# robertknight/rten

Measured on NVIDIA H100. Metric: resnet50_fp32_inferences_per_sec, higher is better.
Workload: dtype f32(tf32 mma, explicit opt-in)

## Files before the change

### rten_b200/csrc/umma_gemm.cu

```cuda
#include <cuda.h>
#include <cuda_runtime.h>

#include <algorithm>
#include <array>
#include <cmath>
#include <vector>
#include <cmath>
#include <cstdint>
#include <cstdio>
#include <cstdlib>

#include "math.cuh"
#include "ptx.cuh"
#include "rowops.h"
#include "umma_gemm.h"
#include "umma_kernel.cuh"

namespace rtb {

typedef CUresult (*EncodeTiledFn)(CUtensorMap*, CUtensorMapDataType, cuuint32_t, void*, const cuuint64_t*,
                                  const cuuint64_t*, const cuuint32_t*, const cuuint32_t*, CUtensorMapInterleave,
                                  CUtensorMapSwizzle, CUtensorMapL2promotion, CUtensorMapFloatOOBfill);

static EncodeTiledFn get_encode(rten_ctx* ctx) {
// ... 38 lines not shown
        long long s = od.strides[i] * esize;
        if (s == 0 || od.dims[i] == 1) s = 16;
        strides[i - 1] = (cuuint64_t)s;
    }
    CUresult r = enc(map, is_f32 ? CU_TENSOR_MAP_DATA_TYPE_FLOAT32 : CU_TENSOR_MAP_DATA_TYPE_UINT8, 4,
                     const_cast<void*>(od.base), dims, strides, b, es, CU_TENSOR_MAP_INTERLEAVE_NONE,
                     CU_TENSOR_MAP_SWIZZLE_128B, CU_TENSOR_MAP_L2_PROMOTION_L2_256B,
                     CU_TENSOR_MAP_FLOAT_OOB_FILL_NONE);
    return r == CUDA_SUCCESS;
}

static void pick_conv_tile(const ConvGeom& g, int& tw, int& th, int& tb) {
    double best = -1.0;
    tw = th = tb = 1;
    for (int w = 1; w <= std::min(g.OW, 128); w++) {
        if (w * g.sx > 256) break;
        for (int h = 1; h <= std::min(g.OH, 128 / w); h++) {
            if (h * g.sy > 256) break;
            int b = std::min(g.B, 128 / (w * h));
            if (b < 1) continue;
            long long tiles = (long long)((g.OW + w - 1) / w) * ((g.OH + h - 1) / h) * ((g.B + b - 1) / b);
            double eff = (double)g.B * g.OH * g.OW / ((double)tiles * 128.0);
            if (eff > best + 1e-9 || (eff > best - 1e-9 && w > tw)) {
                best = eff;
                tw = w;
                th = h;
                tb = b;
            }
        }
    }
}

struct Plan {
    int bn = 32, splitk = 1, nbuf = 1;
};

struct Prepared {
    KParams p;
    uint32_t abox[4], aes[4], bbox_k;
    uint32_t pbox[4], pes[4];
    uint32_t a_rows;
    long long batch;
    OperandDesc od, ord;
    uint32_t dbox[4];
    int tma_store, res_tma;
    int wide;
    int chain_bytes;
    int step;
    int esize, kelems;
};

constexpr int SK_CNT_INTS = 1 << 16;
static int smem_budget_for(int n_stg) { return 227 * 1024 - SMEM_FIXED_BYTES - n_stg * STG_BYTES; }
static int wide_stages(int stage_bytes, int chain_bytes) {
    return std::min(MAX_STAGES, (227 * 1024 - WIDE_SMEM_FIXED_BYTES - chain_bytes) / stage_bytes);
}
static bool is_wide(int bn) { return bn > ACC_STRIDE; }

static Epi pick_epilogue(const GemmLaunch& L, int tma_store, int res_tma, int splitk) {
    const EpilogueDesc& e = L.epi;
    auto aligned = [](const void* ptr) { return (reinterpret_cast<uintptr_t>(ptr) & 15) == 0; };
    bool fast = tma_store && (L.N % 32) == 0 && !getenv("RTEN_B200_NO_FAST") && e.bias_kind != 2 &&
                (e.r == nullptr || res_tma) && (e.bias_kind != 1 || aligned(e.bias));
    if (L.kind == 1)
        fast = fast && (!(e.za || e.za8) || aligned(e.colsum)) && (!e.zb || e.zb_len == 1 || (e.zb_len == L.N && aligned(e.zb))) &&
               (!e.scale || e.scale_len == 1 || (e.scale_len == L.N && aligned(e.scale)));
    if (!fast) return Epi::Generic;
    const bool gelu = e.act > 1;
    if (!getenv("RTEN_B200_NO_PLAIN") && e.act <= 7) {
        if (L.kind == 0 && e.alpha == 1.0f && !e.range && (e.r == nullptr || e.r_scale == 1.0f))
            return gelu ? Epi::PlainF32Gelu : Epi::PlainF32;
        if (L.kind == 1 && e.scale && !e.za && !e.zb && (e.scale_len == 1 || e.scale_len == L.N) && splitk == 1 &&
            (!e.za8 || e.colsum))
            return gelu ? Epi::PlainI8Gelu : Epi::PlainI8;
    }
    return gelu ? Epi::FastGelu : Epi::Fast;
}

static const char* epi_name(Epi v) {
    static const char* const names[] = {"Generic", "Fast", "FastGelu", "PlainF32", "PlainF32Gelu", "PlainI8", "PlainI8Gelu"};
    return names[(int)v];
}

static bool is_plain_f32(Epi v) { return v == Epi::PlainF32 || v == Epi::PlainF32Gelu; }

struct PlanShape {
    long long tiles_n, units_m, tiles, units;
    int kb_per, stage_bytes, stages, n_stg;
};

static bool plan_shape(const Prepared& q, const Plan& pl, PlanShape& ps) {
    const KParams& p = q.p;
    if (pl.splitk < 1) return false;
    if (is_wide(pl.bn)) {
        if ((pl.bn != 128 && pl.bn != 256) || !q.wide || pl.splitk != 1) return false;
        if (pl.bn == 256 && q.p.epi.act > 1) return false;
    } else if (pl.bn < 16 || pl.bn % 32 || pl.bn % q.step) {
        return false;
    }
    if (pl.nbuf < (q.res_tma ? 2 : 1) || pl.nbuf > 4) return false;
    ps.tiles_n = q.chain_bytes ? 1 : (p.N + pl.bn - 1) / pl.bn;
    ps.units_m = p.tiles_m;
    ps.tiles = ps.units_m * ps.tiles_n * q.batch;
    ps.units = ps.tiles * pl.splitk;
    if (ps.units > 0x7FFFFFFFll) return false;
    ps.kb_per = (p.k_blocks + pl.splitk - 1) / pl.splitk;
    if (pl.splitk > 1) {
        if (pl.bn % 32 || (long long)(pl.splitk - 1) * ps.kb_per >= p.k_blocks) return false;
        if (ps.tiles * 2 > SK_CNT_INTS) return false;
    }
    ps.n_stg = 2 * pl.nbuf;
    ps.stage_bytes = A_STAGE_BYTES + pl.bn * KBYTES;
    ps.stages = is_wide(pl.bn) ? wide_stages(ps.stage_bytes, q.chain_bytes) : std::min(MAX_STAGES, smem_budget_for(ps.n_stg) / ps.stage_bytes);
    if (ps.stages < 2) return false;
    return true;
}

static double plan_cost(const Prepared& q, const Plan& pl, const PlanShape& ps, int num_sms) {
    const double active = (double)std::min<long long>(ps.units, num_sms);
    const double waves = std::ceil((double)ps.units / num_sms);
    const double bw = std::min(64.0, 7400.0 / active);
    const double mmas = 4.0;
    const double t_kb = std::max(mmas * std::max(42.0, (double)pl.bn), ps.stage_bytes / bw);
    double t_stage = std::max(t_kb, 320.0 + mmas * 42.0);
    t_stage = std::max(t_stage, 2300.0 / ps.stages);
    const double mainloop = ps.kb_per * t_stage;
    const double epi = is_wide(pl.bn) ? (pl.bn / 32.0) * 400.0 + 600.0 : (pl.bn / 32.0) * 350.0 / 2.0 + 600.0;
    double unit = (is_wide(pl.bn) ? mainloop + epi : std::max(mainloop, epi)) + 1500.0;
    double cost = waves * unit + 2500.0;
    if (pl.splitk > 1) cost += epi * (1.0 + 0.25 * pl.splitk) + 1500.0;

    return cost;
}

static void enumerate_plans(const Prepared& q, int num_sms, std::vector<std::pair<double, Plan>>& out) {
    const KParams& p = q.p;
    const int nmax = (p.N + q.step - 1) / q.step * q.step;
    static const int splits[] = {1, 2, 3, 4, 5, 6, 8, 10, 12, 16};
    for (int bn : {32, 64, 128, 256}) {
        if (bn > nmax && bn != 32) break;
        for (int sk : splits) {
            Plan pl;
            pl.bn = bn;
            pl.splitk = sk;
            if (sk > 1 && p.k_blocks / sk < 4) continue;
            const int kb_per = (p.k_blocks + sk - 1) / sk;
            pl.nbuf = (q.res_tma || kb_per < 24) ? 2 : 1;
            PlanShape ps;
            if (is_wide(bn)) {
                pl.nbuf = 2;
            } else if (pl.nbuf == 2 && !getenv("RTEN_B200_NO_NBUF3")) {
                PlanShape ps2;
                const bool ok2 = plan_shape(q, pl, ps2);
                pl.nbuf = 3;
                if (!plan_shape(q, pl, ps) || (ps.stages < 3 && !(ok2 && ps.stages == ps2.stages))) pl.nbuf = 2;
            }
            if (!plan_shape(q, pl, ps)) continue;
            if (sk > 1 && ps.tiles >= 2 * num_sms) continue;
            if (ps.stages < 2) continue;
            out.emplace_back(plan_cost(q, pl, ps, num_sms), pl);
        }
    }
    std::sort(out.begin(), out.end(), [](const std::pair<double, Plan>& x, const std::pair<double, Plan>& y) {
        return x.first < y.first;
    });
}

static rten_status prepare_launch(rten_ctx* ctx, const GemmLaunch& L, Prepared& q) {
    const int esize = L.kind == 0 ? 4 : 1;
    const int kelems = KBYTES / esize;
    if (!tma_compatible(L.a, esize, 4) || !tma_compatible(L.b, esize, 4)) return RTEN_ERR_UNSUPPORTED_VALUE;
    if (L.M <= 0 || L.N <= 0 || L.K <= 0) return RTEN_ERR_UNSUPPORTED_VALUE;
    q.esize = esize;
    q.kelems = kelems;
    KParams& p = q.p;
    memset(&p, 0, sizeof(p));
    p.M = L.M;
    p.N = L.N;
    p.K = L.K;
    p.z0 = L.z0;
    p.z1 = L.z1;
    p.kelems = kelems;
    p.conv = L.conv;
    p.epi = L.epi;
    p.c_blocks = 1;
    p.kw = 1;
    for (int i = 0; i < 4; i++) q.aes[i] = 1;
    if (L.conv) {
        const ConvGeom& g = L.g;
        pick_conv_tile(g, p.tw, p.th, p.tb);
        p.tiles_x = (g.OW + p.tw - 1) / p.tw;
        p.tiles_y = (g.OH + p.th - 1) / p.th;
        int tiles_b = (g.B + p.tb - 1) / p.tb;
        p.tiles_m = p.tiles_x * p.tiles_y * tiles_b;
        p.OH = g.OH;
        p.OW = g.OW;
        p.Bn = g.B;
        p.sy = g.sy;
        p.sx = g.sx;
        p.dy = g.dy;
        p.dx = g.dx;
        p.pt = g.pt;
        p.pl = g.pl;
// ... 147 lines not shown
    p.stages = ps.stages;
    p.sgn = L.kind == 0 ? 0 : (L.a_signed ? 1 : 0) | (L.b_signed ? 2 : 0);
    if (p.splitk > 1) {
        RTB_TRY(ensure_splitk_counters(ctx));
        if (!ws) RTB_TRY(temp_alloc(ctx, splitk_ws_bytes(ps, pl), &ws));
        p.sk_ws = reinterpret_cast<uint32_t*>(ws);
        p.sk_cnt = reinterpret_cast<int*>(ctx->sk_counters);
    }

    uint32_t bbox[4] = {(uint32_t)q.kelems, (uint32_t)p.bn, 1, 1}, bes[4] = {1, 1, 1, 1}, des[4] = {1, 1, 1, 1};
    TmaMaps m;
    if (!encode_map(ctx, &m.a, L.a, q.esize, L.kind == 0, q.abox, q.aes)) return RTEN_ERR_UNSUPPORTED_VALUE;
    if (!encode_map(ctx, &m.b, L.b, q.esize, L.kind == 0, bbox, bes)) return RTEN_ERR_UNSUPPORTED_VALUE;
    m.d = m.r = m.a2 = m.a_proj = m.b_proj = m.a2_proj = m.w2 = m.z = m.a;
    p.x3_cb = L.x3_cb;
    if (L.x3_cb && !encode_map(ctx, &m.a2, L.a_lo, q.esize, true, q.abox, q.aes)) return RTEN_ERR_UNSUPPORTED_VALUE;
    if (p.kb_proj) {
        p.x3_cb_proj = L.proj.x3_cb;
        if (!encode_map(ctx, &m.a_proj, L.proj.a, 4, true, q.pbox, q.pes) ||
            !encode_map(ctx, &m.b_proj, L.proj.b, 4, true, bbox, bes) ||
            (L.proj.x3_cb && !encode_map(ctx, &m.a2_proj, L.proj.a_lo, 4, true, q.pbox, q.pes)))
            return RTEN_ERR_UNSUPPORTED_VALUE;
    }
    if (p.tma_store && !encode_map(ctx, &m.d, q.od, 4, true, q.dbox, des)) {
        p.tma_store = 0;
        p.res_tma = 0;
        m.d = m.a;
    }
    if (p.res_tma && !encode_map(ctx, &m.r, q.ord, 4, true, q.dbox, des)) {
        p.res_tma = 0;
        m.r = m.a;
    }
    const Epi epi = pick_epilogue(L, p.tma_store, p.res_tma, p.splitk);
    if (epi == Epi::Generic && (L.kind == 1 || L.epi.act > 1)) p.res_tma = 0;
    if (q.chain_bytes) {
        const GemmLaunch::Chain& c = L.chain;
        const uint32_t wbox[4] = {32, (uint32_t)c.N2, 1, 1}, zbox[4] = {32, q.dbox[1], q.dbox[2], q.dbox[3]};
        if (epi != Epi::PlainF32 || (L.epi.r && !p.res_tma) || !encode_map(ctx, &m.w2, c.w, 4, true, wbox, des) ||
            !encode_map(ctx, &m.z, c.z, 4, true, zbox, des))
            return RTEN_ERR_UNSUPPORTED_VALUE;
        p.chain_n2 = c.N2;
        p.chain_passes = (L.N + p.bn - 1) / p.bn;
        p.chain_act = c.act;
        p.chain_bias = c.bias;
    }

    if (verbose)
        fprintf(stderr, "[umma_gemm] kind=%d conv=%d M=%d N=%d K=%d kb=%d kb_proj=%d tiles_m=%d bn=%d splitk=%d units=%d stages=%d tma_store=%d res_tma=%d nbuf=%d box=%dx%dx%d epi=%s%s\n",
                L.kind, L.conv, L.M, L.N, L.K, p.k_blocks, p.kb_proj, p.tiles_m, p.bn, p.splitk, p.units_total, p.stages,
                p.tma_store, p.res_tma, p.nbuf, p.tw, p.th, p.tb, epi_name(epi),
                p.chain_n2 == 64 ? " chain=64" : p.chain_n2 == 128 ? " chain=128" : "");
    if ((is_wide(p.bn) || p.kb_proj || L.epi.bias2) && !is_plain_f32(epi)) return RTEN_ERR_UNSUPPORTED_VALUE;
    const size_t smem_bytes = (size_t)p.stages * p.stage_bytes + q.chain_bytes +
                              (is_wide(p.bn) ? WIDE_SMEM_FIXED_BYTES : ps.n_stg * STG_BYTES + SMEM_FIXED_BYTES);
    using Kernel = void (*)(TmaMaps, KParams);
    static const Kernel narrow[2][7] = {
        {umma_gemm_kernel<0, Epi::Generic>, umma_gemm_kernel<0, Epi::Fast>, umma_gemm_kernel<0, Epi::FastGelu>,
         umma_gemm_kernel<0, Epi::PlainF32>, umma_gemm_kernel<0, Epi::PlainF32Gelu>, nullptr, nullptr},
        {umma_gemm_kernel<1, Epi::Generic>, umma_gemm_kernel<1, Epi::Fast>, umma_gemm_kernel<1, Epi::FastGelu>, nullptr,
         nullptr, umma_gemm_kernel<1, Epi::PlainI8>, umma_gemm_kernel<1, Epi::PlainI8Gelu>}};
    const Kernel kern = !is_wide(p.bn)              ? narrow[L.kind][(int)epi]
                        : p.chain_n2 == 64         ? umma_wide_kernel<Epi::PlainF32, 64>
                        : p.chain_n2 == 128        ? umma_wide_kernel<Epi::PlainF32, 128>
                        : epi == Epi::PlainF32Gelu ? umma_wide_kernel<Epi::PlainF32Gelu>
                                                   : umma_wide_kernel<Epi::PlainF32>;

    const int threads = is_wide(p.bn) ? WIDE_THREADS : NUM_THREADS;
    return launch(ctx, "umma_gemm launch", kern, {std::min(p.units_total, ctx->num_sms), threads, smem_bytes, 227 * 1024, true}, m, p);
}

static std::vector<long long> tune_key(const GemmLaunch& L, const Prepared& q) {
    const EpilogueDesc& e = L.epi;
    std::vector<long long> k = {L.kind, L.conv, L.M, L.N, L.K, L.z0, L.z1, q.tma_store, q.res_tma, e.act, e.bias_kind,
                                e.r != nullptr, (e.za != nullptr || e.za8 != nullptr), e.zb != nullptr, e.scale != nullptr,
                                L.a.strides[1], L.b.strides[1], L.x3_cb};
    if (L.conv) {
        const ConvGeom& g = L.g;
        for (long long v : {g.B, g.H, g.W, g.C, g.OH, g.OW, g.kh, g.kw, g.sy, g.sx, g.dy, g.dx, g.pt, g.pl}) k.push_back(v);
    }
    if (L.proj.C > 0) {
        const GemmLaunch::Projection& pr = L.proj;
        for (int64_t v : {(int64_t)-1, (int64_t)pr.C, (int64_t)pr.stride, (int64_t)pr.x3_cb, pr.a.dims[1], pr.a.dims[2],
                          pr.a.strides[1], pr.a.strides[2], pr.a.strides[3], pr.b.strides[1]})
            k.push_back(v);
    }
    return k;
}

static Plan plan_from_array(const std::array<int, 3>& a) {
    Plan pl;
    pl.bn = a[0];
    pl.splitk = a[1];
    pl.nbuf = a[2];
    return pl;
}

static rten_status launch_tf32x3(rten_ctx* ctx, const GemmLaunch& L0) {
    GemmLaunch L = L0;
    long long d0 = 0, d0p = 0;
    auto split = [&](const OperandDesc& src, OperandDesc& dst, int role, void* into) -> rten_status {
        const long long planes = role == 2 ? 1 : 3;
        long long dims[4], strides[4], n = planes * d0p;
        for (int i = 0; i < 4; i++) {
            dims[i] = (i > 0 && src.strides[i] == 0) ? 1 : src.dims[i];
            strides[i] = src.strides[i];
        }
        for (int i = 1; i < 4; i++) n *= dims[i];
        void* buf = into;
        if (!buf) RTB_TRY(temp_alloc(ctx, (size_t)n * 4, &buf));
        RTB_TRY(launch_tf32x3_split(ctx, (const float*)src.base, (float*)buf, dims, strides, d0p, role));
        dst = src;
        dst.base = buf;
        dst.dims[0] = planes * d0p;
        long long st = planes * d0p;
        for (int i = 1; i < 4; i++) {
            dst.strides[i] = (src.strides[i] == 0 && src.dims[i] > 1) ? 0 : st;
// ... 23 lines not shown
        }
        if (slot && *slot && !getenv("RTEN_B200_X3_NO_CACHE")) {
            b = b0;
            b.base = *slot;
            b.dims[0] = 3 * d0p;
            long long st = 3 * d0p;
            for (int i = 1; i < 4; i++) {
                const long long di = b0.strides[i] == 0 ? 1 : b0.dims[i];
                b.strides[i] = (b0.strides[i] == 0 && b0.dims[i] > 1) ? 0 : st;
                st *= di;
            }
        } else {
            RTB_TRY(split(b0, b, 1, nullptr));
        }
        const bool two_plane = d0 % 32 == 0 && tma_compatible(a0, 4, 4) && !getenv("RTEN_B200_X3_THREE_PLANES");
        if (two_plane && a_lo_base) {
            a_lo = a0;
            a_lo.base = a_lo_base;
            x3_cb = (int)(d0 / 32);
        } else if (two_plane) {
            RTB_TRY(split(a0, a_lo, 2, nullptr));
            x3_cb = (int)(d0 / 32);
        } else {
            RTB_TRY(split(a0, a, 0, nullptr));
        }
        return RTEN_OK;
    };
    RTB_TRY(split_source(L0.a, L0.b, L0.b_x3_slot, L0.a_lo_base, L.a, L.b, L.a_lo, L.x3_cb));
    if (L.conv)
        L.g.C = (int)(3 * d0p);
    L.K = L.conv ? (int)(L0.K / d0 * 3 * d0p) : (int)(3 * d0p);
    L.b_x3_slot = nullptr;
    L.a_lo_base = nullptr;
    if (L0.proj.C > 0) {
        RTB_TRY(split_source(L0.proj.a, L0.proj.b, L0.proj.b_x3_slot, nullptr, L.proj.a, L.proj.b, L.proj.a_lo, L.proj.x3_cb));
        L.proj.C = (int)(3 * d0p);
        L.proj.b_x3_slot = nullptr;
    }
    const int saved = ctx->f32_mode;
    ctx->f32_mode = RTEN_F32_TF32;
    const rten_status st = launch_umma_gemm(ctx, L);
    ctx->f32_mode = saved;
    return st;
}

rten_status launch_umma_gemm(rten_ctx* ctx, const GemmLaunch& L) {
    if (L.chain.N2 > 0) {
        if (L.kind != 0 || ctx->f32_mode != RTEN_F32_TF32 || L.x3_cb || getenv("RTEN_B200_NO_CHAIN"))
            return RTEN_ERR_UNSUPPORTED_VALUE;
        Prepared q;
        RTB_TRY(prepare_launch(ctx, L, q));
        Plan pl;
        pl.bn = 128;
        pl.nbuf = 2;
        return launch_plan(ctx, L, q, pl, getenv("RTEN_B200_VERBOSE") != nullptr);
    }
    if (L.kind == 0 && ctx->f32_mode == RTEN_F32_TF32X3) return launch_tf32x3(ctx, L);
    if (L.conv && L.kind == 0 && L.g.kh * L.g.kw > 1 && !L.x3_cb && !L.proj.C) {
        const rten_status hs = launch_umma_halo_conv(ctx, L);
        if (hs != RTEN_ERR_UNSUPPORTED_VALUE) return hs;
    }
    Prepared q;
    RTB_TRY(prepare_launch(ctx, L, q));
    const bool verbose = getenv("RTEN_B200_VERBOSE") != nullptr;
    const bool forced = getenv("RTEN_B200_FORCE_BN") || getenv("RTEN_B200_FORCE_SPLITK");
    if (!forced && !ctx->tune_cache.empty()) {
        auto hit = ctx->tune_cache.find(tune_key(L, q));
        if (hit != ctx->tune_cache.end()) {
            PlanShape ps;
            if (hit->second[0] < 0) {
                const rten_status hs = launch_umma_halo_conv(ctx, L, hit->second[1], hit->second[2]);
                if (hs != RTEN_ERR_UNSUPPORTED_VALUE) return hs;
            } else
            if (plan_shape(q, plan_from_array(hit->second), ps)) return launch_plan(ctx, L, q, plan_from_array(hit->second), verbose);
            if (verbose) fprintf(stderr, "[umma_gemm] recorded plan no longer valid for this problem: re-planning\n");
            ctx->tune_cache.erase(hit);
        }
    }
    std::vector<std::pair<double, Plan>> cands;
    enumerate_plans(q, ctx->num_sms, cands);
    if (cands.empty()) return RTEN_ERR_UNSUPPORTED_VALUE;
    Plan plan = cands[0].second;

    if (forced) {
        const char* fb = getenv("RTEN_B200_FORCE_BN");
        const char* fs = getenv("RTEN_B200_FORCE_SPLITK");
        bool found = false;
        for (const auto& c : cands) {
            const Plan& x = c.second;
            if (fb && x.bn != atoi(fb)) continue;
            if (fs && x.splitk != atoi(fs)) continue;
            plan = x;
            found = true;
            break;
        }
        if (!found) {
            ctx->forced_misses++;
            if (verbose) fprintf(stderr, "[umma_gemm] no valid plan matches the forced fields: using the model's choice\n");
            if (getenv("RTEN_B200_FORCE_STRICT"))
                return fail(ctx, RTEN_ERR_INVALID_VALUE, "no launch plan matches the forced RTEN_B200_FORCE_* fields");
        } else {
            ctx->forced_hits++;
        }
    } else if (ctx->autotune || !ctx->tune_cache.empty()) {
        const std::vector<long long> key = tune_key(L, q);
        auto it = ctx->tune_cache.find(key);
        PlanShape ps_hit;
// ... 107 lines not shown
```

### rten_b200/csrc/umma_kernel.cuh

```cuda
#pragma once
#include <cuda.h>
#include <cuda_runtime.h>

#include <cstdint>

#include "math.cuh"
#include "ptx.cuh"
#include "umma_gemm.h"

namespace rtb {

constexpr int BM = 128;
constexpr int KBYTES = 128;
constexpr int A_STAGE_BYTES = BM * KBYTES;
constexpr int ACC_STRIDE = 64;
constexpr int PRODUCER_WARP = 12;
constexpr int NUM_THREADS = 416;
constexpr int STG_BYTES = 128 * 128;
constexpr int MAX_STAGES = 8;

struct FastDiv {
    uint32_t d = 1, mul = 0, shr = 0;
    __host__ void set(int div) {
        d = (uint32_t)(div < 1 ? 1 : div);
// ... 46 lines not shown
    EpilogueDesc epi;
};

struct TileCoord {
    int n0;
    int m0;
    int z0, z1;
    int ox0, oy0, b0;
};

__device__ __forceinline__ TileCoord decode_tile(const KParams& p, int t) {
    TileCoord c;
    int n_blk, rest, m_blk, z;
    p.d_tiles_n.divmod(t, rest, n_blk);
    p.d_tiles_m.divmod(rest, z, m_blk);
    c.n0 = n_blk * p.bn;
    c.m0 = m_blk * BM;
    p.d_z0.divmod(z, c.z1, c.z0);
    c.ox0 = c.oy0 = c.b0 = 0;
    if (p.conv) {
        int xt, r2, yt, bt;
        p.d_tiles_x.divmod(m_blk, r2, xt);
        p.d_tiles_y.divmod(r2, bt, yt);
        c.ox0 = xt * p.tw;
        c.oy0 = yt * p.th;
        c.b0 = bt * p.tb;
    }
    return c;
}

__device__ __forceinline__ int4 out_coord(const KParams& p, const TileCoord& tc, int col) {
    return p.conv ? make_int4(tc.n0 + col, tc.ox0, tc.oy0, tc.b0) : make_int4(tc.n0 + col, tc.m0, tc.z0, tc.z1);
}

__device__ __forceinline__ void plain_f32_pair(uint32_t& v0, uint32_t& v1, bool res, float2 rr, float2 bb, bool relu) {
    if (res) add_f32x2(v0, v1, rr.x, rr.y);
    add_f32x2(v0, v1, bb.x, bb.y);
    if (relu) {
        v0 = __float_as_uint(fmaxf(__uint_as_float(v0), 0.0f));
        v1 = __float_as_uint(fmaxf(__uint_as_float(v1), 0.0f));
    }
}

__device__ __forceinline__ float column_bias(const EpilogueDesc& e, int n) {
    const float b = __ldg(e.bias + n);
    return e.bias2 ? __fadd_rn(b, __ldg(e.bias2 + n)) : b;
}

__device__ __forceinline__ void bulk_wait_read(int n) {
    switch (n) {
        case 0: asm volatile("cp.async.bulk.wait_group.read 0;" ::: "memory"); break;
        case 1: asm volatile("cp.async.bulk.wait_group.read 1;" ::: "memory"); break;
        case 2: asm volatile("cp.async.bulk.wait_group.read 2;" ::: "memory"); break;
        default: asm volatile("cp.async.bulk.wait_group.read 3;" ::: "memory"); break;
    }
}

__device__ __forceinline__ int f32_to_ordered(float f) {
    const int i = __float_as_int(f);
    return i >= 0 ? i : i ^ 0x7fffffff;
}
__device__ __forceinline__ void range_commit(int* range, float lo, float hi) {
#pragma unroll
    for (int o = 16; o > 0; o >>= 1) {
        lo = fminf(lo, __shfl_xor_sync(0xffffffffu, lo, o));
        hi = fmaxf(hi, __shfl_xor_sync(0xffffffffu, hi, o));
    }
    if ((threadIdx.x & 31) == 0 && lo <= hi) {
        atomicMin(&range[0], f32_to_ordered(lo));
        atomicMax(&range[1], f32_to_ordered(hi));
    }
}

__device__ __noinline__ float4 act4(float4 x, int act, float alpha, float beta) {
    if (act == 2) {
        gelu_ref_x2(x.x, x.y);
        gelu_ref_x2(x.z, x.w);
        return x;
    }
    x.x = apply_act(x.x, act, alpha, beta);
    x.y = apply_act(x.y, act, alpha, beta);
    x.z = apply_act(x.z, act, alpha, beta);
    x.w = apply_act(x.w, act, alpha, beta);
    return x;
}

__device__ __forceinline__ bool splitk_publish(const KParams& p, int t, int ks, int grp, int q, int lane, uint32_t t_acc,
                                               int* flag, uint32_t acc_smem) {
    const int r = q * 32 + lane;
    const int nchunks = p.bn >> 5;
    for (int c0 = grp * 32; c0 < p.bn; c0 += 64) {
        uint32_t v[32];
        acc_ld(acc_smem, t_acc + c0, v);
        uint32_t* w = p.sk_ws + ((((size_t)t * p.splitk + ks) * nchunks + (c0 >> 5)) << 12) + r;
#pragma unroll
        for (int j = 0; j < 32; j++) __stcg(w + j * 128, v[j]);
    }
    __threadfence();
    asm volatile("bar.sync %0, 128;" ::"r"(1 + grp) : "memory");
    if (q == 0 && lane == 0) {
        int* cnt = p.sk_cnt + t * 2 + grp;
        const int old = atomicAdd(cnt, 1);
        const int last = old == p.splitk - 1;
        if (last) *cnt = 0;
        __threadfence();
        *flag = last;
    }
// ... 215 lines not shown
    L.smem = base + 4096 + ACC_SMEM_BYTES;
    return L;
}

__device__ __forceinline__ void kernel_setup(const SmemLayout& L) {
    const int warp = threadIdx.x >> 5;
    const int lane = threadIdx.x & 31;
    if (warp == PRODUCER_WARP) {
        if (lane < MAX_STAGES) {
            mbar_init(&L.full_bar[lane], 1);
            mbar_init(&L.empty_bar[lane], 4);
        }
        fence_mbar_init();
        __syncwarp();
        asm volatile("bar.arrive 15, %0;" ::"r"(NUM_THREADS) : "memory");
        return;
    }
    if (warp == 1) {
        if (lane < 2)
            mbar_init(&L.acc_full[lane], 128);
        else if (lane < 4)
            mbar_init(&L.acc_empty[lane - 2], 8);
        else if (lane < 12)
            mbar_init(&L.res_bar[lane - 4], 1);
        fence_mbar_init();
    }
    asm volatile("bar.sync 15, %0;" ::"r"(NUM_THREADS) : "memory");
}

template <int KIND, Epi E>
__global__ void __launch_bounds__(NUM_THREADS, 1)
umma_gemm_kernel(const __grid_constant__ TmaMaps m, const __grid_constant__ KParams p) {
    extern __shared__ uint8_t smem_raw[];
    const SmemLayout L = carve_smem(smem_raw);
    if (threadIdx.x == 0) prefetch_maps(m, p);
    kernel_setup(L);
    if (threadIdx.x >> 5 != PRODUCER_WARP) pdl_wait();
    pdl_launch_dependents();
    const int worker = (int)blockIdx.x, n_workers = (int)gridDim.x;
    const int warp = threadIdx.x >> 5;
    if (warp == PRODUCER_WARP) {
        producer_role(p, m, L, worker, n_workers);
    } else if (warp < 4) {
        if (p.bn == 32)
            mma_role<KIND, 32>(p, L, worker, n_workers);
        else
            mma_role<KIND, 64>(p, L, worker, n_workers);
    } else {
        epilogue<KIND, E>(p, L, &m.d, &m.r, worker, n_workers);
    }
}

constexpr int WIDE_THREADS = 384;
constexpr int WIDE_SMEM_FIXED_BYTES = 1024 + 2 * STG_BYTES + 2048;

template <int N>
__device__ __forceinline__ void wgmma_wide(float (&d)[N / 2], uint64_t adesc, uint64_t bdesc) {
    if constexpr (N == 128) wgmma_tf32_n128(d, adesc, bdesc);
    else wgmma_tf32_n256(d, adesc, bdesc);
}

__device__ __forceinline__ void consumers_sync() { asm volatile("bar.sync 1, 256;" ::: "memory"); }

__device__ __forceinline__ int chain_w_bytes(const KParams& p) { return (p.N / 32) * p.chain_n2 * KBYTES; }

template <bool CHAIN>
__device__ __forceinline__ SmemLayout carve_wide_smem(uint8_t* smem_raw, const KParams& p) {
    uint8_t* base = reinterpret_cast<uint8_t*>((reinterpret_cast<uintptr_t>(smem_raw) + 1023) & ~uintptr_t(1023));
    uint8_t* tail = base + (size_t)p.stages * p.stage_bytes + (CHAIN ? chain_w_bytes(p) : 0) + 2 * STG_BYTES;
    SmemLayout L;
    L.smem = base;
    L.full_bar = reinterpret_cast<uint64_t*>(tail);
    L.empty_bar = L.full_bar + MAX_STAGES;
    L.res_bar = L.empty_bar + MAX_STAGES;
    L.w_bar = L.res_bar + 2;
    L.acc_full = L.acc_empty = nullptr;
    L.sk_flag = nullptr;
    L.bias = reinterpret_cast<float*>(tail + 256);
    L.acc_smem = 0;
    return L;
}

template <int N>
__device__ __forceinline__ void wide_main_loop(const KParams& p, const SmemLayout& L, float (&d)[N / 2], int wg, int lane,
                                               int& stage, uint32_t& ring) {
    const uint32_t smem0 = smem_u32(L.smem);
#pragma unroll
    for (int i = 0; i < N / 2; i++) d[i] = 0.0f;
    int prev = -1;
    for (int kb = 0; kb < p.k_blocks; kb++) {
        mbar_wait(&L.full_bar[stage], (ring >> stage) & 1);
        wgmma_fence_operand(d);
        wgmma_fence();
        const uint32_t sa = smem0 + stage * p.stage_bytes;
        const uint64_t adesc = make_kmajor_sw128_desc(sa + wg * (64 * KBYTES));
        const uint64_t bdesc = make_kmajor_sw128_desc(sa + A_STAGE_BYTES);
#pragma unroll
        for (int k = 0; k < 4; k++) wgmma_wide<N>(d, adesc + 2 * k, bdesc + 2 * k);
        wgmma_commit();
        wgmma_fence_operand(d);
        wgmma_wait<1>();
        if (prev >= 0 && lane == 0) mbar_arrive(&L.empty_bar[prev]);
        prev = stage;
        ring ^= 1u << stage;
        if (++stage == p.stages) stage = 0;
    }
    wgmma_wait<0>();
    wgmma_fence_operand(d);
    if (prev >= 0 && lane == 0) mbar_arrive(&L.empty_bar[prev]);
}

template <Epi E, int NA>
__device__ __forceinline__ void stage_chunk(float (&d)[NA], int k, uint8_t* stg, const float* bias, bool valid, bool res,
                                            int act, int row0, int sw, int cq, float alpha = 0.0f, float beta = 0.0f) {
#pragma unroll
    for (int j = 0; j < 4; j++) {
        const int i0 = 16 * k + 4 * j;
        float2* px[2];
#pragma unroll
        for (int h = 0; h < 2; h++)
            px[h] = reinterpret_cast<float2*>(stg + (row0 + 8 * h) * 128 + (((2 * j + (cq >> 1)) ^ sw) << 4) + 8 * (cq & 1));
        if (valid) {
            const float2 bb = *reinterpret_cast<const float2*>(bias + 8 * j + 2 * cq);
#pragma unroll
            for (int h = 0; h < 2; h++) {
                uint32_t v0 = __float_as_uint(d[i0 + 2 * h]), v1 = __float_as_uint(d[i0 + 2 * h + 1]);
                float2 rr = make_float2(0.f, 0.f);
                if (res) rr = *px[h];
                plain_f32_pair(v0, v1, res, rr, bb, act == 1);
                d[i0 + 2 * h] = __uint_as_float(v0);
                d[i0 + 2 * h + 1] = __uint_as_float(v1);
            }
            if (E == Epi::PlainF32Gelu) {
                const float4 g = act4(make_float4(d[i0], d[i0 + 1], d[i0 + 2], d[i0 + 3]), act, alpha, beta);
                d[i0] = g.x;
                d[i0 + 1] = g.y;
                d[i0 + 2] = g.z;
                d[i0 + 3] = g.w;
            }
        }
#pragma unroll
        for (int h = 0; h < 2; h++) *px[h] = make_float2(d[i0 + 2 * h], d[i0 + 2 * h + 1]);
    }
}

template <Epi E, int N>
__device__ __forceinline__ void wide_consumer(const KParams& p, const SmemLayout& L, const CUtensorMap* tma_d,
                                              const CUtensorMap* tma_r, int worker, int n_workers) {
    const int t = threadIdx.x - 128;
    const int wg = t >> 7;
    const int lane = threadIdx.x & 31;
    const int row0 = 64 * wg + 16 * ((t & 127) >> 5) + (lane >> 2);
    const int sw = lane >> 2;
    const int cq = lane & 3;
    const bool issuer = t == 0;
    const EpilogueDesc& e = p.epi;
    uint8_t* const stg0 = L.smem + (size_t)p.stages * p.stage_bytes;
    float* const bias_s = L.bias;
    uint32_t ring = 0, rphase = 0;
    uint32_t ci = 0;
    int stage = 0;
    auto load_residual = [&](const TileCoord& tc, int c0, int buf) {
        uint64_t* rb = &L.res_bar[buf];
        mbar_expect_tx(rb, p.res_tx_bytes);
        const int4 x = out_coord(p, tc, c0);
        tma_load_4d(stg0 + buf * STG_BYTES, tma_r, rb, x.x, x.y, x.z, x.w);
    };
    for (int u = worker; u < p.units_total; u += n_workers) {
        {
            const TileCoord tc = decode_tile(p, u);
            if (t < N) bias_s[t] = (e.bias_kind == 1 && tc.n0 + t < p.N) ? column_bias(e, tc.n0 + t) : 0.0f;
            if (issuer) {
                bulk_wait_read(0);
                if (p.res_tma) load_residual(tc, 0, ci & 1);
            }
        }
        float d[N / 2];
        wide_main_loop<N>(p, L, d, wg, lane, stage, ring);
        const TileCoord tc = decode_tile(p, u);
        consumers_sync();
#pragma unroll
        for (int k = 0; k < N / 32; k++, ci++) {
            const int buf = ci & 1;
            uint8_t* stg = stg0 + buf * STG_BYTES;
            const int nbase = tc.n0 + 32 * k;
            if (issuer) {
                bulk_wait_read(0);
                if (p.res_tma && k + 1 < N / 32) load_residual(tc, 32 * (k + 1), buf ^ 1);
            }
            if (p.res_tma) {
                mbar_wait(&L.res_bar[buf], (rphase >> buf) & 1);
                rphase ^= 1u << buf;
            }
            stage_chunk<E>(d, k, stg, bias_s + 32 * k, nbase < p.N, p.res_tma, e.act, row0, sw, cq, e.act_alpha, e.act_beta);
            fence_proxy_async();
            consumers_sync();
            if (issuer) {
                const int4 x = out_coord(p, tc, 32 * k);
                tma_store_4d(tma_d, stg, x.x, x.y, x.z, x.w);
                asm volatile("cp.async.bulk.commit_group;" ::: "memory");
            }
        }
    }
    if (issuer) asm volatile("cp.async.bulk.wait_group.read 0;" ::: "memory");
}

template <int N2>
__device__ __forceinline__ void wide_chain_consumer(const KParams& p, const SmemLayout& L, const TmaMaps& m, int worker,
                                                    int n_workers) {
    constexpr int N = 128;
    const int t = threadIdx.x - 128;
    const int wg = t >> 7;
    const int lane = threadIdx.x & 31;
    const int row0 = 64 * wg + 16 * ((t & 127) >> 5) + (lane >> 2);
    const int sw = lane >> 2;
    const int cq = lane & 3;
    const bool issuer = t == 0;
    const EpilogueDesc& e = p.epi;
    const uint32_t w2 = smem_u32(L.smem) + p.stages * p.stage_bytes;
    uint8_t* const stg0 = L.smem + (size_t)p.stages * p.stage_bytes + chain_w_bytes(p);
    float* const bias_s = L.bias;
    uint32_t ring = 0, rphase = 0;
    uint32_t ci = 0;
    int stage = 0;
    auto load_residual = [&](const TileCoord& tc, int c0, int buf) {
        uint64_t* rb = &L.res_bar[buf];
        mbar_expect_tx(rb, p.res_tx_bytes);
        const int4 x = out_coord(p, tc, c0);
        tma_load_4d(stg0 + buf * STG_BYTES, &m.r, rb, x.x, x.y, x.z, x.w);
    };
    auto chunk_barrier = [&](float (&acc2)[N2 / 2]) {
        wgmma_wait<0>();
        wgmma_fence_operand(acc2);
        if (issuer) bulk_wait_read(0);
        fence_proxy_async();
        consumers_sync();
    };
    mbar_wait(L.w_bar, 0);
    for (int u = worker; u < p.units_total; u += n_workers) {
        {
            const TileCoord tc = decode_tile(p, u);
            if (t < p.N) bias_s[t] = e.bias_kind == 1 ? column_bias(e, t) : 0.0f;
            if (t < N2) bias_s[256 + t] = p.chain_bias ? __ldg(p.chain_bias + t) : 0.0f;
            if (issuer && p.res_tma) load_residual(tc, 0, ci & 1);
        }
        float acc2[N2 / 2];
#pragma unroll
        for (int i = 0; i < N2 / 2; i++) acc2[i] = 0.0f;
        for (int pass = 0; pass < p.chain_passes; pass++) {
            float d[N / 2];
            wide_main_loop<N>(p, L, d, wg, lane, stage, ring);
            const TileCoord tc = decode_tile(p, u);
            consumers_sync();
#pragma unroll
            for (int k = 0; k < N / 32; k++) {
                const int c0 = N * pass + 32 * k;
                if (c0 >= p.N) break;
                const int buf = ci & 1;
                uint8_t* stg = stg0 + buf * STG_BYTES;
                if (p.res_tma) {
                    mbar_wait(&L.res_bar[buf], (rphase >> buf) & 1);
                    rphase ^= 1u << buf;
                }
                stage_chunk<Epi::PlainF32>(d, k, stg, bias_s + c0, true, p.res_tma, e.act, row0, sw, cq);
                chunk_barrier(acc2);
                if (issuer) {
                    const int4 x = out_coord(p, tc, c0);
                    tma_store_4d(&m.d, stg, x.x, x.y, x.z, x.w);
                    asm volatile("cp.async.bulk.commit_group;" ::: "memory");
                    if (p.res_tma && c0 + 32 < p.N) load_residual(tc, c0 + 32, buf ^ 1);
                }
                wgmma_fence();
                const uint64_t adesc = make_kmajor_sw128_desc(smem_u32(stg) + wg * (64 * KBYTES));
                const uint64_t bdesc = make_kmajor_sw128_desc(w2 + (c0 / 32) * (N2 * KBYTES));
#pragma unroll
                for (int kk = 0; kk < 4; kk++) {
                    if constexpr (N2 == 64) wgmma_tf32_n64(acc2, adesc + 2 * kk, bdesc + 2 * kk);
                    else wgmma_tf32_n128(acc2, adesc + 2 * kk, bdesc + 2 * kk);
                }
                wgmma_commit();
                wgmma_fence_operand(acc2);
                ci++;
            }
        }
        wgmma_wait<0>();
        wgmma_fence_operand(acc2);
        const TileCoord tc = decode_tile(p, u);
#pragma unroll
        for (int k = 0; k < N2 / 32; k++, ci++) {
            uint8_t* stg = stg0 + (ci & 1) * STG_BYTES;
            stage_chunk<Epi::PlainF32>(acc2, k, stg, bias_s + 256 + 32 * k, true, false, p.chain_act, row0, sw, cq);
            chunk_barrier(acc2);
            if (issuer) {
                tma_store_4d(&m.z, stg, 32 * k, tc.ox0, tc.oy0, tc.b0);
                asm volatile("cp.async.bulk.commit_group;" ::: "memory");
            }
        }
    }
    if (issuer) asm volatile("cp.async.bulk.wait_group.read 0;" ::: "memory");
}

template <Epi E, int CHAIN_N2 = 0>
__global__ void __launch_bounds__(WIDE_THREADS, 1)
umma_wide_kernel(const __grid_constant__ TmaMaps m, const __grid_constant__ KParams p) {
    extern __shared__ uint8_t smem_raw[];
    const SmemLayout L = carve_wide_smem<(CHAIN_N2 > 0)>(smem_raw, p);
    const int warp = threadIdx.x >> 5;
    const int lane = threadIdx.x & 31;
    if (threadIdx.x == 0) {
        prefetch_maps(m, p);
        if constexpr (CHAIN_N2 > 0) {
            tma_prefetch_desc(&m.w2);
            tma_prefetch_desc(&m.z);
        }
    }
    if (warp == 1) {
        if (lane < MAX_STAGES) {
            mbar_init(&L.full_bar[lane], 1);
            mbar_init(&L.empty_bar[lane], 8);
        } else if (lane < MAX_STAGES + (CHAIN_N2 > 0 ? 3 : 2)) {
            mbar_init(&L.res_bar[lane - MAX_STAGES], 1);
        }
        fence_mbar_init();
    }
    __syncthreads();
    if (warp >= 4) pdl_wait();
    pdl_launch_dependents();
    if (warp < 4) {
        asm volatile("setmaxnreg.dec.sync.aligned.u32 56;");
        if (warp == 0) producer_role<(CHAIN_N2 > 0)>(p, m, L, (int)blockIdx.x, (int)gridDim.x);
    } else {
        asm volatile("setmaxnreg.inc.sync.aligned.u32 224;");
        if constexpr (CHAIN_N2 > 0) {
            wide_chain_consumer<CHAIN_N2>(p, L, m, (int)blockIdx.x, (int)gridDim.x);
        } else {
            if (E == Epi::PlainF32Gelu || p.bn == 128)
                wide_consumer<E, 128>(p, L, &m.d, &m.r, (int)blockIdx.x, (int)gridDim.x);
            else
                wide_consumer<E, 256>(p, L, &m.d, &m.r, (int)blockIdx.x, (int)gridDim.x);
        }
    }
}

}
```

Before: 16830.

## Add deeper staging ring for wide-kernel epilogue with residual prefetch

Replaces the fixed double-buffered epilogue staging in the wide GEMM kernel with a configurable ring of up to 8 buffers. Residual TMA loads are issued several chunks ahead, and stores wait only until a slack count of groups is still pending, not for all of them. The planner now enumerates nbuf values for wide tiles on residual convolutions and charges the staging memory against pipeline stages. The aim is to overlap residual loads and output stores with the epilogue math, at the cost of shared memory taken from mainloop stages and more complex barrier bookkeeping.

```diff
diff --git a/rten_b200/csrc/umma_gemm.cu b/rten_b200/csrc/umma_gemm.cu
--- a/rten_b200/csrc/umma_gemm.cu
+++ b/rten_b200/csrc/umma_gemm.cu
@@ -114,8 +114,8 @@
 
 constexpr int SK_CNT_INTS = 1 << 16;
 static int smem_budget_for(int n_stg) { return 227 * 1024 - SMEM_FIXED_BYTES - n_stg * STG_BYTES; }
-static int wide_stages(int stage_bytes, int chain_bytes) {
-    return std::min(MAX_STAGES, (227 * 1024 - WIDE_SMEM_FIXED_BYTES - chain_bytes) / stage_bytes);
+static int wide_stages(int stage_bytes, int chain_bytes, int nbuf) {
+    return std::min(MAX_STAGES, (227 * 1024 - WIDE_SMEM_FIXED_BYTES - nbuf * STG_BYTES - chain_bytes) / stage_bytes);
 }
 static bool is_wide(int bn) { return bn > ACC_STRIDE; }
 
@@ -160,7 +160,8 @@
     } else if (pl.bn < 16 || pl.bn % 32 || pl.bn % q.step) {
         return false;
     }
-    if (pl.nbuf < (q.res_tma ? 2 : 1) || pl.nbuf > 4) return false;
+    if (is_wide(pl.bn) ? (pl.nbuf < 2 || pl.nbuf > MAX_WIDE_NBUF) : (pl.nbuf < (q.res_tma ? 2 : 1) || pl.nbuf > 4))
+        return false;
     ps.tiles_n = q.chain_bytes ? 1 : (p.N + pl.bn - 1) / pl.bn;
     ps.units_m = p.tiles_m;
     ps.tiles = ps.units_m * ps.tiles_n * q.batch;
@@ -173,7 +174,7 @@
     }
     ps.n_stg = 2 * pl.nbuf;
     ps.stage_bytes = A_STAGE_BYTES + pl.bn * KBYTES;
-    ps.stages = is_wide(pl.bn) ? wide_stages(ps.stage_bytes, q.chain_bytes) : std::min(MAX_STAGES, smem_budget_for(ps.n_stg) / ps.stage_bytes);
+    ps.stages = is_wide(pl.bn) ? wide_stages(ps.stage_bytes, q.chain_bytes, pl.nbuf) : std::min(MAX_STAGES, smem_budget_for(ps.n_stg) / ps.stage_bytes);
     if (ps.stages < 2) return false;
     return true;
 }
@@ -187,7 +188,9 @@
     double t_stage = std::max(t_kb, 320.0 + mmas * 42.0);
     t_stage = std::max(t_stage, 2300.0 / ps.stages);
     const double mainloop = ps.kb_per * t_stage;
-    const double epi = is_wide(pl.bn) ? (pl.bn / 32.0) * 400.0 + 600.0 : (pl.bn / 32.0) * 350.0 / 2.0 + 600.0;
+    const double wide_chunk =
+        q.res_tma && q.p.conv ? std::max(250.0, 800.0 / (pl.nbuf - wide_store_slack(pl.nbuf, true))) : 400.0;
+    const double epi = is_wide(pl.bn) ? (pl.bn / 32.0) * wide_chunk + 600.0 : (pl.bn / 32.0) * 350.0 / 2.0 + 600.0;
     double unit = (is_wide(pl.bn) ? mainloop + epi : std::max(mainloop, epi)) + 1500.0;
     double cost = waves * unit + 2500.0;
     if (pl.splitk > 1) cost += epi * (1.0 + 0.25 * pl.splitk) + 1500.0;
@@ -210,7 +213,12 @@
             pl.nbuf = (q.res_tma || kb_per < 24) ? 2 : 1;
             PlanShape ps;
             if (is_wide(bn)) {
-                pl.nbuf = 2;
+                for (int nb : {2, 4, 8}) {
+                    if (nb > 2 && !(q.res_tma && p.conv)) break;
+                    pl.nbuf = nb;
+                    if (plan_shape(q, pl, ps)) out.emplace_back(plan_cost(q, pl, ps, num_sms), pl);
+                }
+                continue;
             } else if (pl.nbuf == 2 && !getenv("RTEN_B200_NO_NBUF3")) {
                 PlanShape ps2;
                 const bool ok2 = plan_shape(q, pl, ps2);
@@ -464,7 +472,7 @@
                 p.chain_n2 == 64 ? " chain=64" : p.chain_n2 == 128 ? " chain=128" : "");
     if ((is_wide(p.bn) || p.kb_proj || L.epi.bias2) && !is_plain_f32(epi)) return RTEN_ERR_UNSUPPORTED_VALUE;
     const size_t smem_bytes = (size_t)p.stages * p.stage_bytes + q.chain_bytes +
-                              (is_wide(p.bn) ? WIDE_SMEM_FIXED_BYTES : ps.n_stg * STG_BYTES + SMEM_FIXED_BYTES);
+                              (is_wide(p.bn) ? p.nbuf * STG_BYTES + WIDE_SMEM_FIXED_BYTES : ps.n_stg * STG_BYTES + SMEM_FIXED_BYTES);
     using Kernel = void (*)(TmaMaps, KParams);
     static const Kernel narrow[2][7] = {
         {umma_gemm_kernel<0, Epi::Generic>, umma_gemm_kernel<0, Epi::Fast>, umma_gemm_kernel<0, Epi::FastGelu>,
@@ -474,6 +482,8 @@
     const Kernel kern = !is_wide(p.bn)              ? narrow[L.kind][(int)epi]
                         : p.chain_n2 == 64         ? umma_wide_kernel<Epi::PlainF32, 64>
                         : p.chain_n2 == 128        ? umma_wide_kernel<Epi::PlainF32, 128>
+                        : p.nbuf > 2 || p.conv     ? (epi == Epi::PlainF32Gelu ? umma_wide_kernel<Epi::PlainF32Gelu, 0, true>
+                                                                               : umma_wide_kernel<Epi::PlainF32, 0, true>)
                         : epi == Epi::PlainF32Gelu ? umma_wide_kernel<Epi::PlainF32Gelu>
                                                    : umma_wide_kernel<Epi::PlainF32>;
 
@@ -603,7 +613,9 @@
         RTB_TRY(prepare_launch(ctx, L, q));
         Plan pl;
         pl.bn = 128;
-        pl.nbuf = 2;
+        PlanShape ps;
+        for (pl.nbuf = q.res_tma ? MAX_WIDE_NBUF : 2; pl.nbuf > 2; pl.nbuf--)
+            if (plan_shape(q, pl, ps)) break;
         return launch_plan(ctx, L, q, pl, getenv("RTEN_B200_VERBOSE") != nullptr);
     }
     if (L.kind == 0 && ctx->f32_mode == RTEN_F32_TF32X3) return launch_tf32x3(ctx, L);
diff --git a/rten_b200/csrc/umma_kernel.cuh b/rten_b200/csrc/umma_kernel.cuh
--- a/rten_b200/csrc/umma_kernel.cuh
+++ b/rten_b200/csrc/umma_kernel.cuh
@@ -122,7 +122,10 @@
         case 0: asm volatile("cp.async.bulk.wait_group.read 0;" ::: "memory"); break;
         case 1: asm volatile("cp.async.bulk.wait_group.read 1;" ::: "memory"); break;
         case 2: asm volatile("cp.async.bulk.wait_group.read 2;" ::: "memory"); break;
-        default: asm volatile("cp.async.bulk.wait_group.read 3;" ::: "memory"); break;
+        case 3: asm volatile("cp.async.bulk.wait_group.read 3;" ::: "memory"); break;
+        case 4: asm volatile("cp.async.bulk.wait_group.read 4;" ::: "memory"); break;
+        case 5: asm volatile("cp.async.bulk.wait_group.read 5;" ::: "memory"); break;
+        default: asm volatile("cp.async.bulk.wait_group.read 6;" ::: "memory"); break;
     }
 }
 
@@ -444,7 +447,49 @@
 }
 
 constexpr int WIDE_THREADS = 384;
-constexpr int WIDE_SMEM_FIXED_BYTES = 1024 + 2 * STG_BYTES + 2048;
+constexpr int MAX_WIDE_NBUF = 8;
+constexpr int WIDE_SMEM_FIXED_BYTES = 1024 + 2048;
+
+__host__ __device__ constexpr int wide_store_slack(int nbuf, bool res) { return res ? (nbuf > 2 ? 1 : 0) : nbuf - 2; }
+
+struct WideRing {
+    uint8_t* stg0;
+    int nb, ahead, per_unit, res_chunks;
+    int buf = 0;
+    uint32_t ci = 0, rphase = 0;
+    uint32_t rq = 0;
+    int rbuf = 0, rk = 0, ru;
+    __device__ WideRing(uint8_t* s, int nbuf, int slack, int chunks, int res, int worker)
+        : stg0(s), nb(nbuf), ahead(nbuf - slack), per_unit(chunks), res_chunks(res), ru(worker) {}
+    __device__ __forceinline__ uint8_t* stg() const { return stg0 + buf * STG_BYTES; }
+    __device__ __forceinline__ void load(const KParams& p, const CUtensorMap* tma_r, uint64_t* res_bar, const TileCoord& tc,
+                                         int col, int b) {
+        const int4 x = out_coord(p, tc, col);
+        mbar_expect_tx(&res_bar[b], p.res_tx_bytes);
+        tma_load_4d(stg0 + b * STG_BYTES, tma_r, &res_bar[b], x.x, x.y, x.z, x.w);
+    }
+    __device__ __forceinline__ void request(const KParams& p, const CUtensorMap* tma_r, uint64_t* res_bar, uint32_t limit,
+                                            int n_workers) {
+        if (!res_chunks) return;
+        while (rq < limit && ru < p.units_total) {
+            if (rk < res_chunks) load(p, tma_r, res_bar, decode_tile(p, ru), 32 * rk, rbuf);
+            rq++;
+            if (++rbuf == nb) rbuf = 0;
+            if (++rk == per_unit) {
+                rk = 0;
+                ru += n_workers;
+            }
+        }
+    }
+    __device__ __forceinline__ void wait_residual(uint64_t* res_bar) {
+        mbar_wait(&res_bar[buf], (rphase >> buf) & 1);
+        rphase ^= 1u << buf;
+    }
+    __device__ __forceinline__ void next() {
+        ci++;
+        if (++buf == nb) buf = 0;
+    }
+};
 
 template <int N>
 __device__ __forceinline__ void wgmma_wide(float (&d)[N / 2], uint64_t adesc, uint64_t bdesc) {
@@ -459,13 +504,13 @@
 template <bool CHAIN>
 __device__ __forceinline__ SmemLayout carve_wide_smem(uint8_t* smem_raw, const KParams& p) {
     uint8_t* base = reinterpret_cast<uint8_t*>((reinterpret_cast<uintptr_t>(smem_raw) + 1023) & ~uintptr_t(1023));
-    uint8_t* tail = base + (size_t)p.stages * p.stage_bytes + (CHAIN ? chain_w_bytes(p) : 0) + 2 * STG_BYTES;
+    uint8_t* tail = base + (size_t)p.stages * p.stage_bytes + (CHAIN ? chain_w_bytes(p) : 0) + (size_t)p.nbuf * STG_BYTES;
     SmemLayout L;
     L.smem = base;
     L.full_bar = reinterpret_cast<uint64_t*>(tail);
     L.empty_bar = L.full_bar + MAX_STAGES;
     L.res_bar = L.empty_bar + MAX_STAGES;
-    L.w_bar = L.res_bar + 2;
+    L.w_bar = L.res_bar + MAX_WIDE_NBUF;
     L.acc_full = L.acc_empty = nullptr;
     L.sk_flag = nullptr;
     L.bias = reinterpret_cast<float*>(tail + 256);
@@ -536,7 +581,7 @@
     }
 }
 
-template <Epi E, int N>
+template <Epi E, int N, bool RING>
 __device__ __forceinline__ void wide_consumer(const KParams& p, const SmemLayout& L, const CUtensorMap* tma_d,
                                               const CUtensorMap* tma_r, int worker, int n_workers) {
     const int t = threadIdx.x - 128;
@@ -547,24 +592,19 @@
     const int cq = lane & 3;
     const bool issuer = t == 0;
     const EpilogueDesc& e = p.epi;
-    uint8_t* const stg0 = L.smem + (size_t)p.stages * p.stage_bytes;
     float* const bias_s = L.bias;
-    uint32_t ring = 0, rphase = 0;
-    uint32_t ci = 0;
+    uint32_t ring = 0;
     int stage = 0;
-    auto load_residual = [&](const TileCoord& tc, int c0, int buf) {
-        uint64_t* rb = &L.res_bar[buf];
-        mbar_expect_tx(rb, p.res_tx_bytes);
-        const int4 x = out_coord(p, tc, c0);
-        tma_load_4d(stg0 + buf * STG_BYTES, tma_r, rb, x.x, x.y, x.z, x.w);
-    };
+    const int slack = wide_store_slack(p.nbuf, p.res_tma);
+    WideRing rg(L.smem + (size_t)p.stages * p.stage_bytes, p.nbuf, slack, N / 32, p.res_tma ? N / 32 : 0, worker);
     for (int u = worker; u < p.units_total; u += n_workers) {
         {
             const TileCoord tc = decode_tile(p, u);
             if (t < N) bias_s[t] = (e.bias_kind == 1 && tc.n0 + t < p.N) ? column_bias(e, tc.n0 + t) : 0.0f;
-            if (issuer) {
+            if (RING && issuer) rg.request(p, tma_r, L.res_bar, rg.ci + rg.ahead - 1, n_workers);
+            if (!RING && issuer) {
                 bulk_wait_read(0);
-                if (p.res_tma) load_residual(tc, 0, ci & 1);
+                if (p.res_tma) rg.load(p, tma_r, L.res_bar, tc, 0, rg.buf);
             }
         }
         float d[N / 2];
@@ -572,26 +612,26 @@
         const TileCoord tc = decode_tile(p, u);
         consumers_sync();
 #pragma unroll
-        for (int k = 0; k < N / 32; k++, ci++) {
-            const int buf = ci & 1;
-            uint8_t* stg = stg0 + buf * STG_BYTES;
+        for (int k = 0; k < N / 32; k++) {
             const int nbase = tc.n0 + 32 * k;
-            if (issuer) {
+            if (RING && issuer) {
+                bulk_wait_read(slack);
+                rg.request(p, tma_r, L.res_bar, rg.ci + rg.ahead, n_workers);
+            }
+            if (!RING && issuer) {
                 bulk_wait_read(0);
-                if (p.res_tma && k + 1 < N / 32) load_residual(tc, 32 * (k + 1), buf ^ 1);
-            }
-            if (p.res_tma) {
-                mbar_wait(&L.res_bar[buf], (rphase >> buf) & 1);
-                rphase ^= 1u << buf;
-            }
-            stage_chunk<E>(d, k, stg, bias_s + 32 * k, nbase < p.N, p.res_tma, e.act, row0, sw, cq, e.act_alpha, e.act_beta);
+                if (p.res_tma && k + 1 < N / 32) rg.load(p, tma_r, L.res_bar, tc, 32 * (k + 1), rg.buf ^ 1);
+            }
+            if (p.res_tma) rg.wait_residual(L.res_bar);
+            stage_chunk<E>(d, k, rg.stg(), bias_s + 32 * k, nbase < p.N, p.res_tma, e.act, row0, sw, cq, e.act_alpha, e.act_beta);
             fence_proxy_async();
             consumers_sync();
             if (issuer) {
                 const int4 x = out_coord(p, tc, 32 * k);
-                tma_store_4d(tma_d, stg, x.x, x.y, x.z, x.w);
+                tma_store_4d(tma_d, rg.stg(), x.x, x.y, x.z, x.w);
                 asm volatile("cp.async.bulk.commit_group;" ::: "memory");
             }
+            rg.next();
         }
     }
     if (issuer) asm volatile("cp.async.bulk.wait_group.read 0;" ::: "memory");
@@ -610,32 +650,29 @@
     const bool issuer = t == 0;
     const EpilogueDesc& e = p.epi;
     const uint32_t w2 = smem_u32(L.smem) + p.stages * p.stage_bytes;
-    uint8_t* const stg0 = L.smem + (size_t)p.stages * p.stage_bytes + chain_w_bytes(p);
     float* const bias_s = L.bias;
-    uint32_t ring = 0, rphase = 0;
-    uint32_t ci = 0;
+    uint32_t ring = 0;
     int stage = 0;
-    auto load_residual = [&](const TileCoord& tc, int c0, int buf) {
-        uint64_t* rb = &L.res_bar[buf];
-        mbar_expect_tx(rb, p.res_tx_bytes);
-        const int4 x = out_coord(p, tc, c0);
-        tma_load_4d(stg0 + buf * STG_BYTES, &m.r, rb, x.x, x.y, x.z, x.w);
-    };
+    const int slack = wide_store_slack(p.nbuf, p.res_tma);
+    WideRing rg(L.smem + (size_t)p.stages * p.stage_bytes + chain_w_bytes(p), p.nbuf, slack, p.N / 32 + N2 / 32,
+                p.res_tma ? p.N / 32 : 0, worker);
     auto chunk_barrier = [&](float (&acc2)[N2 / 2]) {
         wgmma_wait<0>();
         wgmma_fence_operand(acc2);
-        if (issuer) bulk_wait_read(0);
+        if (issuer) bulk_wait_read(slack);
         fence_proxy_async();
         consumers_sync();
     };
+    auto store_chunk = [&](const CUtensorMap* map, int4 x) {
+        tma_store_4d(map, rg.stg(), x.x, x.y, x.z, x.w);
+        asm volatile("cp.async.bulk.commit_group;" ::: "memory");
+        rg.request(p, &m.r, L.res_bar, rg.ci + rg.ahead, n_workers);
+    };
     mbar_wait(L.w_bar, 0);
     for (int u = worker; u < p.units_total; u += n_workers) {
-        {
-            const TileCoord tc = decode_tile(p, u);
-            if (t < p.N) bias_s[t] = e.bias_kind == 1 ? column_bias(e, t) : 0.0f;
-            if (t < N2) bias_s[256 + t] = p.chain_bias ? __ldg(p.chain_bias + t) : 0.0f;
-            if (issuer && p.res_tma) load_residual(tc, 0, ci & 1);
-        }
+        if (t < p.N) bias_s[t] = e.bias_kind == 1 ? column_bias(e, t) : 0.0f;
+        if (t < N2) bias_s[256 + t] = p.chain_bias ? __ldg(p.chain_bias + t) : 0.0f;
+        if (issuer) rg.request(p, &m.r, L.res_bar, rg.ci + rg.ahead - 1, n_workers);
         float acc2[N2 / 2];
 #pragma unroll
         for (int i = 0; i < N2 / 2; i++) acc2[i] = 0.0f;
@@ -648,22 +685,12 @@
             for (int k = 0; k < N / 32; k++) {
                 const int c0 = N * pass + 32 * k;
                 if (c0 >= p.N) break;
-                const int buf = ci & 1;
-                uint8_t* stg = stg0 + buf * STG_BYTES;
-                if (p.res_tma) {
-                    mbar_wait(&L.res_bar[buf], (rphase >> buf) & 1);
-                    rphase ^= 1u << buf;
-                }
-                stage_chunk<Epi::PlainF32>(d, k, stg, bias_s + c0, true, p.res_tma, e.act, row0, sw, cq);
+                if (p.res_tma) rg.wait_residual(L.res_bar);
+                stage_chunk<Epi::PlainF32>(d, k, rg.stg(), bias_s + c0, true, p.res_tma, e.act, row0, sw, cq);
                 chunk_barrier(acc2);
-                if (issuer) {
-                    const int4 x = out_coord(p, tc, c0);
-                    tma_store_4d(&m.d, stg, x.x, x.y, x.z, x.w);
-                    asm volatile("cp.async.bulk.commit_group;" ::: "memory");
-                    if (p.res_tma && c0 + 32 < p.N) load_residual(tc, c0 + 32, buf ^ 1);
-                }
+                if (issuer) store_chunk(&m.d, out_coord(p, tc, c0));
                 wgmma_fence();
-                const uint64_t adesc = make_kmajor_sw128_desc(smem_u32(stg) + wg * (64 * KBYTES));
+                const uint64_t adesc = make_kmajor_sw128_desc(smem_u32(rg.stg()) + wg * (64 * KBYTES));
                 const uint64_t bdesc = make_kmajor_sw128_desc(w2 + (c0 / 32) * (N2 * KBYTES));
 #pragma unroll
                 for (int kk = 0; kk < 4; kk++) {
@@ -672,27 +699,24 @@
                 }
                 wgmma_commit();
                 wgmma_fence_operand(acc2);
-                ci++;
+                rg.next();
             }
         }
         wgmma_wait<0>();
         wgmma_fence_operand(acc2);
         const TileCoord tc = decode_tile(p, u);
 #pragma unroll
-        for (int k = 0; k < N2 / 32; k++, ci++) {
-            uint8_t* stg = stg0 + (ci & 1) * STG_BYTES;
-            stage_chunk<Epi::PlainF32>(acc2, k, stg, bias_s + 256 + 32 * k, true, false, p.chain_act, row0, sw, cq);
+        for (int k = 0; k < N2 / 32; k++) {
+            stage_chunk<Epi::PlainF32>(acc2, k, rg.stg(), bias_s + 256 + 32 * k, true, false, p.chain_act, row0, sw, cq);
             chunk_barrier(acc2);
-            if (issuer) {
-                tma_store_4d(&m.z, stg, 32 * k, tc.ox0, tc.oy0, tc.b0);
-                asm volatile("cp.async.bulk.commit_group;" ::: "memory");
-            }
+            if (issuer) store_chunk(&m.z, make_int4(32 * k, tc.ox0, tc.oy0, tc.b0));
+            rg.next();
         }
     }
     if (issuer) asm volatile("cp.async.bulk.wait_group.read 0;" ::: "memory");
 }
 
-template <Epi E, int CHAIN_N2 = 0>
+template <Epi E, int CHAIN_N2 = 0, bool RING = false>
 __global__ void __launch_bounds__(WIDE_THREADS, 1)
 umma_wide_kernel(const __grid_constant__ TmaMaps m, const __grid_constant__ KParams p) {
     extern __shared__ uint8_t smem_raw[];
@@ -710,7 +734,7 @@
         if (lane < MAX_STAGES) {
             mbar_init(&L.full_bar[lane], 1);
             mbar_init(&L.empty_bar[lane], 8);
-        } else if (lane < MAX_STAGES + (CHAIN_N2 > 0 ? 3 : 2)) {
+        } else if (lane < MAX_STAGES + MAX_WIDE_NBUF + (CHAIN_N2 > 0 ? 1 : 0)) {
             mbar_init(&L.res_bar[lane - MAX_STAGES], 1);
         }
         fence_mbar_init();
@@ -727,11 +751,11 @@
             wide_chain_consumer<CHAIN_N2>(p, L, m, (int)blockIdx.x, (int)gridDim.x);
         } else {
             if (E == Epi::PlainF32Gelu || p.bn == 128)
-                wide_consumer<E, 128>(p, L, &m.d, &m.r, (int)blockIdx.x, (int)gridDim.x);
+                wide_consumer<E, 128, RING>(p, L, &m.d, &m.r, (int)blockIdx.x, (int)gridDim.x);
             else
-                wide_consumer<E, 256>(p, L, &m.d, &m.r, (int)blockIdx.x, (int)gridDim.x);
-        }
-    }
-}
-
-}
+                wide_consumer<E, 256, RING>(p, L, &m.d, &m.r, (int)blockIdx.x, (int)gridDim.x);
+        }
+    }
+}
+
+}
```

New measurement: 17110, median of 6. 1.7% higher.
